# TobyBoyne/bark

Measured on AMD Instinct MI355X. Metric: forest-Gram + Cholesky MLL evals/sec at N=4096, 50 trees, higher is better.
Workload: dtype f64; 1 GPU; c3: N=4096 d=8 m=50, 256 prior forest samples per GPU (BASELINE configs[2]; sharding of configs[3]), noise U[0.05,0.15), mcmc_record_mll convention; N=4096, d=8, trees=50, forests_per_gpu=256, forests_total=256, chunk=256, parallelism=samples/1, launched_by=bench.py, device_wait=on

## Files before the change

### bark_amd/csrc/chol.hip

```cpp
#include <atomic>
#include <cmath>
#include <cstdlib>
#include <mutex>
#include <type_traits>
#include <vector>

#include "common.h"

namespace bark {

int walk_one_hot(const void *packed, const bark_pack_info *info, const double *X, int64_t N, int64_t d, int words,
                 uint32_t *out, int32_t *fault, hipStream_t stream);
int walk_codes(const void *packed, const bark_pack_info *info, const double *X, int64_t N, int64_t d, uint32_t *out,
               int32_t *fault, hipStream_t stream);
int leafspace_prepare(const uint32_t *codes, int W, int npad, unsigned long long *planes, int R, int Rpad,
                      const double *noise, const double *scale, int m, int bc, double *A, long ld, long bstride,
                      const double *y, int N, double *yz, double *accum, int32_t *info, hipStream_t s);
int leafspace_sumsq(const double *y, int N, double *out, hipStream_t s);
int leafspace_predict(const uint32_t *ccodes, int W, int cpad, int C, const double *w, const double *Minv, int R,
                      const double *noise, const double *scale, int m, int bc, double *mu, double *var, hipStream_t s);
int leafspace_inverse(const uint32_t *codes, int W, int npad, int N, const double *Minv, const double *w, int R,
                      const double *y, const double *noise, const double *scale, int m, int bc, double *Wm, double *kinv,
                      double *kinv_y, hipStream_t s);
int leafspace_finish(const double *accum, const double *yy, const double *noise, const double *scale, int m, int bc, int N,
// ... 58 lines not shown
#ifndef BARK_DIAG_WAVES8
#define BARK_DIAG_WAVES8 1
#endif
constexpr int DIAG8_MAX_BC = 256;
#ifndef BARK_WALK_IN_KERNEL
#define BARK_WALK_IN_KERNEL 1
#endif
#ifndef BARK_TWO_BLOCK
#define BARK_TWO_BLOCK 1
#endif
#ifndef BARK_TWO_MIN_BC
#define BARK_TWO_MIN_BC 1
#endif
constexpr int TWO_MIN_BC = BARK_TWO_MIN_BC, TWO_MAX_BC = 384, TWO_ANY_BC_MAX_N = 224;
#ifndef BARK_MULTI_BLOCK
#define BARK_MULTI_BLOCK 1
#endif
#ifndef BARK_MB_MIN_BC4
#define BARK_MB_MIN_BC4 112
#endif
#ifndef BARK_MB_MIN_BC3
#define BARK_MB_MIN_BC3 80
#endif
#ifndef BARK_MB_MIN_BC5
#define BARK_MB_MIN_BC5 144
#endif
constexpr int MB_MIN_BC4 = BARK_MB_MIN_BC4, MB_MIN_BC3 = BARK_MB_MIN_BC3, MB_MIN_BC5 = BARK_MB_MIN_BC5;
constexpr int MB_CUS = 256;
inline bool mb_chunk_ok(int nrb, int64_t bc) {
    const int64_t rounds = (bc + MB_CUS - 1) / MB_CUS;
    if (bc < (nrb <= 3 ? MB_MIN_BC3 : nrb == 4 ? MB_MIN_BC4 : MB_MIN_BC5)) return false;
    if (rounds <= 1) return true;
    return nrb <= 4 ? bc * 10 >= rounds * MB_CUS * 7 : bc * 5 >= rounds * MB_CUS * 4;
}
inline size_t mb_lds_bytes(int nW, int nrb) {
    return (size_t)(NBLK * SB * SB + 2 * NB + 8 + 2 * nrb * NB + 3 * MB_STAGE) * sizeof(double) + (size_t)nW * nrb * NB * sizeof(uint32_t);
}
#ifndef BARK_PIPE_MIN_NRB
#define BARK_PIPE_MIN_NRB 8
#endif
constexpr int PIPE_MIN_NRB = BARK_PIPE_MIN_NRB;
#ifndef BARK_PLAIN_CHUNK_MULTIPLE
#define BARK_PLAIN_CHUNK_MULTIPLE 256
#endif
constexpr int PLAIN_CHUNK_MULTIPLE = BARK_PLAIN_CHUNK_MULTIPLE;
#ifndef BARK_PLAIN_MIN_NRB
#define BARK_PLAIN_MIN_NRB 16
#endif
#ifndef BARK_PIPE_SYRK_MODE
#define BARK_PIPE_SYRK_MODE 2
#endif
#ifndef BARK_PLAIN_PAIRS
#define BARK_PLAIN_PAIRS 1
#endif
#ifndef BARK_PLAIN_SYRK_MODE
#define BARK_PLAIN_SYRK_MODE 2
#endif
constexpr int PLAIN_MIN_NRB = BARK_PLAIN_MIN_NRB;
#ifndef BARK_SOLVE_NARROW_MAX_WGS
#define BARK_SOLVE_NARROW_MAX_WGS 256
#endif
#ifndef BARK_PIPE_NARROW_MAX_WGS
#define BARK_PIPE_NARROW_MAX_WGS 256
#endif
constexpr long SOLVE_NARROW_MAX_WGS = BARK_SOLVE_NARROW_MAX_WGS, PIPE_NARROW_MAX_WGS = BARK_PIPE_NARROW_MAX_WGS;
#ifndef BARK_SOLVE_DIRECT_MAX_WGS
#define BARK_SOLVE_DIRECT_MAX_WGS 512
#endif
constexpr long SOLVE_DIRECT_MAX_WGS = BARK_SOLVE_DIRECT_MAX_WGS;

#ifndef BARK_DEVWAIT_MAX_BC
#define BARK_DEVWAIT_MAX_BC 32
#endif
constexpr int DEVWAIT_MAX_BC = BARK_DEVWAIT_MAX_BC;

struct Layout {
    int64_t npad, cpad, ncols, ld, W;
    bool splitk;
    size_t off_A, off_W, off_yz, off_acc, off_sync, off_leafx, off_leafc, off_slab, total;
};

inline size_t align256(size_t x) { return (x + 255) & ~(size_t)255; }

Layout make_layout(int64_t N, int64_t C, int64_t m, int64_t Bc) {
    Layout L;
    L.npad = round_up(N, NB);
    L.cpad = C > 0 ? round_up(C, NB) : 0;
    L.ncols = L.npad + L.cpad;
    L.ld = L.ncols + 16;
    L.W = MAX_LEAF_WORDS;
    size_t o = 0;
    L.off_A = o;
    o = align256(o + (size_t)Bc * L.npad * L.ld * sizeof(double));
    L.off_W = o;
    o = align256(o + (size_t)Bc * W_STRIDE * sizeof(double));
    L.off_yz = o;
    o = align256(o + (size_t)Bc * L.npad * sizeof(double));
    L.off_acc = o;
    o = align256(o + (size_t)Bc * 2 * sizeof(double));
    L.off_sync = o;
    o = align256(o + 64);
    L.off_leafx = o;
    o = align256(o + (size_t)Bc * L.W * L.npad * sizeof(uint32_t));
    L.off_leafc = o;
    o = align256(o + (size_t)Bc * L.W * L.cpad * sizeof(uint32_t));
    L.off_slab = o;
// ... 106 lines not shown
                if (hipEventRecord(res->rejoin[i], hs[i]) == hipSuccess) (void)hipStreamWaitEvent(main, res->rejoin[i], 0);
            }
        touched = 0;
        (void)hipGetLastError();
    }
    ~Sweep() {
        for (hipEvent_t e : ev) (void)hipEventDestroy(e);
    }

    int mark_on(hipStream_t s) {
        if (!timed) return BARK_OK;
        hipEvent_t e;
        BARK_HIP_CHECK(hipEventCreate(&e));
        ev.push_back(e);
        BARK_HIP_CHECK(hipEventRecord(e, s));
        return BARK_OK;
    }

    int launch_rows(hipStream_t st, int j, int kdone, int n_right, int n_tiles, int syrk) {
        if (syrk == 2 && n_tiles != n_right + 1) syrk = 0;
        const unsigned diag_wgs = (unsigned)(NXCD * ((p.Bc + NXCD - 1) / NXCD));
        const unsigned grid = syrk == 2 ? xcd_grid(n_right, p.Bc) + diag_wgs : xcd_grid(n_tiles, p.Bc);
        const dim3 g(grid), blk(THREADS);
        if (!fused)
            hipLaunchKernelGGL(row_kernel<0>, g, blk, GEMM_LDS, st, p, j, kdone, n_right, n_tiles, syrk);
        else if (rep == REP_BITS)
            hipLaunchKernelGGL(row_kernel<1 + REP_BITS>, g, blk, GEMM_LDS, st, p, j, kdone, n_right, n_tiles, syrk);
        else if (rep == REP_BYTES7)
            hipLaunchKernelGGL(row_kernel<1 + REP_BYTES7>, g, blk, GEMM_LDS, st, p, j, kdone, n_right, n_tiles, syrk);
        else
            hipLaunchKernelGGL(row_kernel<1 + REP_BYTES8>, g, blk, GEMM_LDS, st, p, j, kdone, n_right, n_tiles, syrk);
        BARK_LAUNCH_CHECK();
        panel_flops += 2.0 * NB * NB * (double)(kdone * NB) * ((double)n_right + (n_tiles > n_right ? (syrk ? 36.0 / 64.0 : 1.0) : 0.0)) * (double)p.Bc;
        return BARK_OK;
    }

    int launch_row_pair(hipStream_t st, int j) {
        const int nA = ncb - j - 1, nB = nA - 1, n_sq = nA + nB, n_syrk = 1 + ((j + 2 < nrb) ? 1 : 0);
        const unsigned grid = xcd_grid(n_sq, p.Bc) + (unsigned)(n_syrk * NXCD * ((p.Bc + NXCD - 1) / NXCD));
        const dim3 g(grid), blk(THREADS);
        if (!fused)
            hipLaunchKernelGGL(row_kernel<0>, g, blk, GEMM_LDS, st, p, j, j, nA, n_sq, 4);
        else if (rep == REP_BITS)
            hipLaunchKernelGGL(row_kernel<1 + REP_BITS>, g, blk, GEMM_LDS, st, p, j, j, nA, n_sq, 4);
        else if (rep == REP_BYTES7)
            hipLaunchKernelGGL(row_kernel<1 + REP_BYTES7>, g, blk, GEMM_LDS, st, p, j, j, nA, n_sq, 4);
        else
            hipLaunchKernelGGL(row_kernel<1 + REP_BYTES8>, g, blk, GEMM_LDS, st, p, j, j, nA, n_sq, 4);
        BARK_LAUNCH_CHECK();
        panel_flops += 2.0 * NB * NB * (double)(j * NB) * ((double)n_sq + n_syrk * 36.0 / 64.0) * (double)p.Bc;
        return BARK_OK;
    }

    int step_paired(int j) {
        hipStream_t s = main, ps = panel;
        const int bc = p.Bc, n_right = ncb - j - 1;
        const bool even = (j & 1) == 0, pair = even && j + 1 < nrb;
        int r;
        const bool has_rows = even && (pair || n_right > 0) && (j >= 1 || fused);
        if (has_rows) {
            BARK_HIP_CHECK(hipEventRecord(res->events[6 * j], s));
            if ((r = after(ps, res->events[6 * j]))) return r;
        }
        const int nkb = j == 0 ? 0 : (even ? 2 : 1);
        const bool deferred = !even;
        if ((r = launch_diag(j, nkb, deferred && n_right > 0, -2, j + 1))) return r;
        if (has_rows) {
            if (timed) panel_marks.push_back(ev.size());
            if ((r = mark_on(ps))) return r;
            if (pair) {
                if ((r = launch_row_pair(ps, j))) return r;
            } else if ((r = launch_rows(ps, j, j, n_right, n_right, 0))) {
                return r;
            }
            if ((r = mark_on(ps))) return r;
            if ((r = join(6 * j + 1))) return r;
        }
        if (n_right > 0) {
            if (timed) solve_marks.push_back(ev.size());
            if ((r = mark_on(s))) return r;
            const dim3 g(xcd_grid(n_right, bc)), blk(THREADS);
            if (deferred)
                hipLaunchKernelGGL(solve_kernel<1>, g, blk, GEMM_LDS, s, p, j, n_right);
            else
                hipLaunchKernelGGL(solve_kernel<0>, g, blk, GEMM_LDS, s, p, j, n_right);
            BARK_LAUNCH_CHECK();
            if ((r = mark_on(s))) return r;
            solve_flops += ((deferred ? 32.0 : 0.0) + 18.0) / 32.0 * 2.0 * NB * NB * (double)NB * (double)n_right * (double)bc;
        }
        return BARK_OK;
    }

    int publish(hipStream_t st, int slot, int value) {
        touch(st);
        hipLaunchKernelGGL(sync_publish_kernel, dim3(1), dim3(1), 0, st, p.sync, slot, value);
        BARK_LAUNCH_CHECK();
        return BARK_OK;
    }

    int gate(hipStream_t st, int value) {
        touch(st);
        hipLaunchKernelGGL(sync_gate_kernel, dim3(1), dim3(1), 0, st, p.sync, 3, value);
        BARK_LAUNCH_CHECK();
        return BARK_OK;
    }

    bool walk_in_kernel(const bark_pack_info *sub, int64_t d) const {
        return BARK_WALK_IN_KERNEL && nrb == 1 && BARK_DIAG_WAVES8 && p.Bc <= DIAG8_MAX_BC &&
               ((size_t)p.N * (d | 1) + 2 + (size_t)sub->m * sub->stride * 2) * sizeof(double) <= (size_t)NBLK * SB * SB * sizeof(double);
    }
    int launch_one_block(const double *y, double *mll, int32_t *fault, int include_2pi, const void *packed_c, const bark_pack_info *sub,
                         const double *X, int64_t d) {
        OneBlock ob{y, mll, fault, include_2pi, rep};
        if (walk_in_kernel(sub, d)) {
            ob.nodes = static_cast<const uint4 *>(packed_c);
            ob.X = X;
            ob.fault_w = fault;
            ob.stride = (int)sub->stride;
            ob.m = (int)sub->m;
            ob.max_depth = (int)sub->max_depth;
            ob.d = (int)d;
        }
        const size_t lds_bytes = DIAG_LDS + (size_t)p.nW * NB * sizeof(uint32_t);
        const bool w8 = BARK_DIAG_WAVES8 && p.Bc <= DIAG8_MAX_BC;
        if (nrb >= 3) {
            hipLaunchKernelGGL(multi_block_kernel, dim3((unsigned)p.Bc), dim3(512), mb_lds_bytes(p.nW, nrb), main, p, ob);
        } else if (nrb == 2) {
            const size_t lds2 = DIAG_LDS + (size_t)p.nW * 2 * NB * sizeof(uint32_t) + 2 * NB * sizeof(double);
            if (w8)
                hipLaunchKernelGGL(two_block_kernel<8>, dim3((unsigned)p.Bc), dim3(512), lds2, main, p, ob);
            else
                hipLaunchKernelGGL(two_block_kernel<4>, dim3((unsigned)p.Bc), dim3(THREADS), lds2, main, p, ob);
        } else if (w8) {
            hipLaunchKernelGGL((diag_kernel<true, 8>), dim3((unsigned)p.Bc), dim3(512), lds_bytes, main, p, 0, 0, 0, -2, 0, ob, 0);
        } else {
            hipLaunchKernelGGL((diag_kernel<true, 4>), dim3((unsigned)p.Bc), dim3(THREADS), lds_bytes, main, p, 0, 0, 0, -2, 0, ob, 0);
        }
        BARK_LAUNCH_CHECK();
        return BARK_OK;
    }

    int launch_diag(int j, int nkb, int want_g = 0, int wait_slot = -2, int wait_value = 0) {
        int r;
        if (timed) diag_marks.push_back(ev.size());
        if ((r = mark_on(main))) return r;
        const bool exclusive = p.Bc <= DIAG_EXCLUSIVE_MAX_BC && !lookahead(j + 1);
        int publish = wait_slot >= -1 ? 1 : 0;
        if (pre_update && nkb > 0) {
            hipLaunchKernelGGL(diag_pre_kernel, dim3(NBLK / (THREADS / 64), (unsigned)p.Bc), dim3(THREADS), 0, main, p, j, nkb, publish);
            BARK_LAUNCH_CHECK();
            nkb = 0;
            publish = 0;
        }
        const OneBlock fin = (fin_mll && j == nrb_steps - 1 && wait_slot < 0) ? OneBlock{nullptr, fin_mll, fin_fault, fin_2pi, rep} : OneBlock{};
        if (fin.mll) finished = true;
        if (exclusive && BARK_DIAG_WAVES8)
            hipLaunchKernelGGL((diag_kernel<false, 8>), dim3((unsigned)p.Bc), dim3(512), DIAG_LDS_EXCLUSIVE, main, p, j, nkb, want_g, wait_slot,
                               wait_value, fin, publish);
        else
            hipLaunchKernelGGL((diag_kernel<false, 4>), dim3((unsigned)p.Bc), dim3(THREADS), exclusive ? DIAG_LDS_EXCLUSIVE : DIAG_LDS, main, p, j, nkb,
                               want_g, wait_slot, wait_value, fin, publish);
        BARK_LAUNCH_CHECK();
        return mark_on(main);
    }

    int fork(int slot) {
        if (panel == main) return BARK_OK;
        BARK_HIP_CHECK(hipEventRecord(res->events[slot], main));
        return after(panel, res->events[slot]);
    }
    int join(int slot) {
        if (panel == main) return BARK_OK;
        BARK_HIP_CHECK(hipEventRecord(res->events[slot], panel));
        BARK_HIP_CHECK(hipStreamWaitEvent(main, res->events[slot], 0));
        joined(panel);
        return BARK_OK;
    }

    int split_factor(int j, int nkb, int slots = SPLITK_SLOTS) const {
        const int n_tiles = (ncb - j - 1) + ((j + 1 < nrb) ? 1 : 0);
        if (!splitk || j < 1 || n_tiles <= 0 || n_tiles * p.Bc >= SPLITK_SLOTS / 2 || nkb < 1) return 1;
        int S = slots / (n_tiles * p.Bc);
        if (slots != SPLITK_SLOTS) {
            S = (2 * slots + n_tiles * p.Bc) / (2 * n_tiles * p.Bc);
            while (S > 1 && S * n_tiles * p.Bc > SPLITK_SLOTS) --S;
        }
        if (S < 1) S = 1;
        int cap = nkb;
        if (slots == SPLITK_SLOTS && (long)n_tiles * p.Bc * nkb * SPLIT_FINE <= SPLIT_FINE_MAX_WGS) cap = nkb * SPLIT_FINE;
        if (S > cap) S = cap;
        if (S > SPLITK_MAX) S = SPLITK_MAX;
        return S;
    }
    bool lookahead(int j) const {
        if (la_stream == nullptr || j < 2 || j >= nrb_steps || split_factor(j, j) <= 1) return false;
        const long n_tiles = (ncb - j - 1) + ((j + 1 < nrb) ? 1 : 0);
        return n_tiles * p.Bc * (long)(j - 1) >= LA_MIN_WORK;
    }
    int la_slots(int j) const {
        const long n_tiles = (ncb - j - 1) + ((j + 1 < nrb) ? 1 : 0);
        return n_tiles * p.Bc * (long)(j - 1) >= LA_BULK_WORK ? LA_SLOTS : LA_SLOTS_CHAIN;
    }
    double *slab_set(int j) const { return slabs + (size_t)(j & 1) * SLAB_SET_TILES * NB * NB; }

    int launch_split(hipStream_t st, int j, int kb_lo, int kb_hi, int S, int s_off, int S_tot, int t_off = 0, int nt = -1) {
        const int n_right = ncb - j - 1, n_all = n_right + ((j + 1 < nrb) ? 1 : 0);
        if (nt < 0) nt = n_all - t_off;
        hipLaunchKernelGGL(panel_split_kernel, dim3(xcd_grid(nt * S, p.Bc)), dim3(THREADS), GEMM_LDS, st, p, j, n_right, t_off, nt,
                           kb_lo, kb_hi, S, s_off, S_tot, slab_set(j));
        BARK_LAUNCH_CHECK();
        panel_flops += 2.0 * NB * NB * (double)((kb_hi - kb_lo) * NB) * (double)nt * (double)p.Bc;
        return BARK_OK;
    }
// ... 806 lines not shown
```

### bark_amd/csrc/chol_diag.h

```cpp
#pragma once
#include <type_traits>

#include "chol_tiles.h"

namespace bark {
namespace {

constexpr int SB = 16;
constexpr int NSB = NB / SB;
constexpr int NBLK = NSB * (NSB + 1) / 2;
constexpr int NSB_ROWS = NSB;

__device__ __forceinline__ int blk_off(int rb, int cb) { return (rb * NSB - (rb * (rb - 1)) / 2 + (cb - rb)) * SB * SB; }
__device__ __forceinline__ double &s_at(double *S, int r, int c) {
    return S[blk_off(r >> 4, c >> 4) + (r & 15) * SB + (c & 15)];
}

__device__ __forceinline__ void mfma_tn(f64x4 &acc, const double *X, int ldx, const double *Y, int ldy, int lr, int lk) {
#pragma unroll
    for (int kk = 0; kk < SB / 4; ++kk)
        acc = __builtin_amdgcn_mfma_f64_16x16x4f64(X[(kk * 4 + lk) * ldx + lr], Y[(kk * 4 + lk) * ldy + lr], acc, 0, 0, 0);
}
__device__ __forceinline__ void mfma_nn(f64x4 &acc, const double *X, int ldx, const double *Y, int ldy, int lr, int lk) {
#pragma unroll
// ... 326 lines not shown
                for (int blk = 0; blk < 8; ++blk)
                    if (blk >= W) fr[blk] = st[(kk * 4 + lk) * LDS_LD + blk * 16 + lr];
#pragma unroll
                for (int i = LO; i < HI; ++i) acc[i] = __builtin_amdgcn_mfma_f64_16x16x4f64(fr[T::rb[i]], fr[T::cb[i]], acc[i], 0, 0, 0);
            }
            asm volatile("s_waitcnt vmcnt(0)" ::: "memory");
            __syncthreads();
        }
    }
#pragma unroll
    for (int i = LO; i < HI; ++i) {
        double *blk = S + blk_off(T::rb[i], T::cb[i]);
#pragma unroll
        for (int v = 0; v < 4; ++v) blk[(lk + 4 * v) * SB + lr] = pre[i][v] - acc[i][v];
    }
}

__device__ __forceinline__ void diag_g(const double *__restrict__ Up, long ld, const double *S, double *__restrict__ Gb, int wave_u,
                                    int lr, int lk) {
#pragma unroll 1
    for (int h = 0; h < 2; ++h) {
        const int kr = wave_u * 2 + h;
        const double *urow = Up + (size_t)(kr * SB + lr) * ld + lk;
        f64x4 g[NSB];
#pragma unroll
        for (int cbk = 0; cbk < NSB; ++cbk) g[cbk] = (f64x4){0.0, 0.0, 0.0, 0.0};
        double a[4], an[4];
#pragma unroll
        for (int q4 = 0; q4 < 4; ++q4) a[q4] = urow[q4 * 4];
#pragma unroll
        for (int rbk = 0; rbk < NSB; ++rbk) {
            if (rbk + 1 < NSB) {
#pragma unroll
                for (int q4 = 0; q4 < 4; ++q4) an[q4] = urow[(rbk + 1) * SB + q4 * 4];
            }
#pragma unroll
            for (int cbk = rbk; cbk < NSB; ++cbk) {
                const double *wb = S + blk_off(rbk, cbk);
#pragma unroll
                for (int q4 = 0; q4 < 4; ++q4)
                    g[cbk] = __builtin_amdgcn_mfma_f64_16x16x4f64(a[q4], wb[(q4 * 4 + lk) * SB + lr], g[cbk], 0, 0, 0);
            }
#pragma unroll
            for (int q4 = 0; q4 < 4; ++q4) a[q4] = an[q4];
            __builtin_amdgcn_sched_barrier(0);
        }
#pragma unroll
        for (int cbk = 0; cbk < NSB; ++cbk)
#pragma unroll
            for (int v = 0; v < 4; ++v) Gb[(size_t)(kr * SB + lk + 4 * v) * NB + cbk * SB + lr] = -g[cbk][v];
    }
}

__device__ __forceinline__ f64x4 frag_transpose(const f64x4 &a, int lr, int lk) {
    f64x4 d = {0.0, 0.0, 0.0, 0.0};
#pragma unroll
    for (int kk = 0; kk < SB / 4; ++kk) d = __builtin_amdgcn_mfma_f64_16x16x4f64(a[kk], (lk + 4 * kk == lr) ? 1.0 : 0.0, d, 0, 0, 0);
    return d;
}

template <int L>
__device__ __forceinline__ f64x4 x_entry(f64x4 (&xt)[L], f64x4 &tacc, int rb, int kb, int nsb, const double *S, const double *dblk,
                                         int lr, int lk) {
    auto term = [&](f64x4 &t, int k, int col, const f64x4 &xf) {
        const double *ub = S + blk_off(k, col);
#pragma unroll
        for (int kk = 0; kk < SB / 4; ++kk) t = __builtin_amdgcn_mfma_f64_16x16x4f64(ub[(kk * 4 + lk) * SB + lr], xf[kk], t, 0, 0, 0);
    };
    if (kb == rb + 1) {
        const double *w = S + blk_off(rb, rb);
        f64x4 wk;
#pragma unroll
        for (int v = 0; v < 4; ++v) wk[v] = w[(lk + 4 * v) * SB + lr];
        xt[0] = frag_transpose(wk, lr, lk);
        tacc = (f64x4){0.0, 0.0, 0.0, 0.0};
    }
    f64x4 t = tacc;
#pragma unroll
    for (int d = 0; d < L; ++d)
        if (rb + d == kb - 1) term(t, kb - 1, kb, xt[d]);
    f64x4 x = {0.0, 0.0, 0.0, 0.0};
#pragma unroll
    for (int kk = 0; kk < SB / 4; ++kk) x = __builtin_amdgcn_mfma_f64_16x16x4f64(dblk[(kk * 4 + lk) * SB + lr], t[kk], x, 0, 0, 0);
    x = -x;
#pragma unroll
    for (int d = 1; d < L; ++d)
        if (rb + d == kb) xt[d] = x;
    if (kb + 1 < nsb) {
        f64x4 tn = {0.0, 0.0, 0.0, 0.0};
#pragma unroll
        for (int d = 0; d < L; ++d)
            if (rb + d < kb) term(tn, rb + d, kb + 1, xt[d]);
        tacc = tn;
    }
    return x;
}

template <int Q, int STRIDE = 3>
__device__ __forceinline__ void c_group(double *S, int kb, int n, int i0, int lr, int lk) {
    const double *a[Q], *b[Q];
    double *dd[Q];
#pragma unroll
    for (int qq = 0; qq < Q; ++qq) {
        int r = 0, rem = i0 + STRIDE * qq + 1;
        while (rem >= n - r) {
            rem -= n - r;
// ... 327 lines not shown
        const double *prev = Ab + (size_t)(j - nkb) * NB * p.ld + (size_t)j * NB;
        const int wsel = __builtin_amdgcn_readfirstlane(wave);
        if (ONE && NW == 8) {
            switch (wsel) {
                case 0: mb_update<0, 0, 5>(prev, p.ld, 0, lds, S, wsel, lane, q.lr, q.lk, p, b, ob.rep, codes, NB, 0); break;
                case 1: mb_update<1, 0, 5>(prev, p.ld, 0, lds, S, wsel, lane, q.lr, q.lk, p, b, ob.rep, codes, NB, 0); break;
                case 2: mb_update<2, 0, 5>(prev, p.ld, 0, lds, S, wsel, lane, q.lr, q.lk, p, b, ob.rep, codes, NB, 0); break;
                case 3: mb_update<3, 0, 5>(prev, p.ld, 0, lds, S, wsel, lane, q.lr, q.lk, p, b, ob.rep, codes, NB, 0); break;
                case 4: mb_update<0, 5, 9>(prev, p.ld, 0, lds, S, wsel, lane, q.lr, q.lk, p, b, ob.rep, codes, NB, 0); break;
                case 5: mb_update<1, 5, 9>(prev, p.ld, 0, lds, S, wsel, lane, q.lr, q.lk, p, b, ob.rep, codes, NB, 0); break;
                case 6: mb_update<2, 5, 9>(prev, p.ld, 0, lds, S, wsel, lane, q.lr, q.lk, p, b, ob.rep, codes, NB, 0); break;
                default: mb_update<3, 5, 9>(prev, p.ld, 0, lds, S, wsel, lane, q.lr, q.lk, p, b, ob.rep, codes, NB, 0); break;
            }
        } else if (wsel == 0)
            diag_update<0, ONE>(tile, p.ld, prev, nkb, lds, S, lane, q.lr, q.lk, p, b, ob.rep, codes);
        else if (wsel == 1)
            diag_update<1, ONE>(tile, p.ld, prev, nkb, lds, S, lane, q.lr, q.lk, p, b, ob.rep, codes);
        else if (wsel == 2)
            diag_update<2, ONE>(tile, p.ld, prev, nkb, lds, S, lane, q.lr, q.lk, p, b, ob.rep, codes);
        else if (NW == 4 || wsel == 3)
            diag_update<3, ONE>(tile, p.ld, prev, nkb, lds, S, lane, q.lr, q.lk, p, b, ob.rep, codes);
        else
            for (int a = (nkb > 1 ? 2 : nkb) * (1 + NB / BK); a > 0; --a) __syncthreads();
    }
    __syncthreads();

    const int lr = q.lr, lk = q.lk;
    const int wave_u = __builtin_amdgcn_readfirstlane(wave);
    const int nsb = one ? (p.N + SB - 1) / SB : NSB;
    DIAG_STAMP(1);
    if (NW == 8)
        factor_tile8<ONE>(S, nsb, copy_only, wave_u, lane, lr, lk, logsum, pacc, bad);
    else
        factor_tile<ONE>(S, nsb, copy_only, wave_u, lane, lr, lk, logsum, pacc, bad);
    DIAG_STAMP(2);

    double *Wb = w_block(p, b);
    auto write_w = [&](int t) {
        const int half = __builtin_amdgcn_readfirstlane(t >> 7), e = 2 * (t & 127), r = e >> 4, c = e & 15;
        int cnt = 0;
#pragma unroll
        for (int rbk = 0; rbk < NSB; ++rbk)
#pragma unroll
            for (int cbk = rbk; cbk < NSB; ++cbk, ++cnt)
                if ((cnt & 1) == half)
                    *reinterpret_cast<f64x2 *>(Wb + (size_t)(rbk * SB + r) * NB + cbk * SB + c) =
                        *reinterpret_cast<const f64x2 *>(S + blk_off(rbk, cbk) + e);
    };
    if (!one && NW == 4) write_w(tid);

    DIAG_STAMP(3);
    if (want_g && (NW == 4 || wave_u < 4))
        diag_g(Ab + (size_t)(j - 1) * NB * p.ld + (size_t)j * NB, p.ld, S, p.W + (size_t)b * W_STRIDE, wave_u, lr, lk);

    DIAG_STAMP(4);
    double *yb = p.yz + (size_t)b * p.nrb * NB + (size_t)j * NB;
    if (tid < NB) vec[tid] = y_in;
    __syncthreads();
    {
        const int c = tid & (NB - 1), half = tid >> 7, cbk = c >> 4, cc = c & 15;
        double part = 0.0;
#pragma unroll
        for (int i = 0; i < NSB / 2; ++i) {
            const int rbk = half * (NSB / 2) + i;
            if (rbk <= cbk && (NW == 4 || half < 2)) {
                const double *col = S + blk_off(rbk, cbk) + cc;
#pragma unroll
                for (int rr = 0; rr < SB; ++rr) part = fma(col[rr * SB], vec[rbk * SB + rr], part);
            }
        }
        if (half == 1) vec[NB + c] = part;
        __syncthreads();
        double zz = 0.0;
        if (!half) {
            const double z = part + vec[NB + c];
            if (!one) yb[c] = z;
            zz = z * z;
        }
#pragma unroll
        for (int off = 32; off > 0; off >>= 1) zz += __shfl_xor(zz, off);
        if (lane == 0) red[wave] = zz;
    }
    __syncthreads();
    DIAG_STAMP(5);
    if (!one && NW == 8 && tid >= THREADS) write_w(tid - THREADS);
    if (tid == 0 && one) {
        double v = -(red[0] + red[1]) - 2.0 * logsum;
        if (ob.include_2pi) v = v - (double)p.N * log(2.0 * M_PI);
        ob.mll[b] = 0.5 * v;
        p.info[b] = *ob.fault ? -1 : (bad ? bad : 0);
    } else if (tid == 0) {
        p.accum[(size_t)b * 2 + 0] = acc_quad + (red[0] + red[1]);
        p.accum[(size_t)b * 2 + 1] = acc_logdet + 2.0 * logsum;
        int code = (bad && info_in == 0) ? j * NB + bad : 0;
        if (wait_slot >= 0) {
            const unsigned long long t0 = __builtin_amdgcn_s_memrealtime();
            const int32_t *flag = p.sync + wait_slot;
            bool ok = true;
            while (__hip_atomic_load(flag, __ATOMIC_RELAXED, __HIP_MEMORY_SCOPE_AGENT) < wait_value) {
                if (__hip_atomic_load(p.sync + 2, __ATOMIC_RELAXED, __HIP_MEMORY_SCOPE_AGENT) != 0) {
                    ok = false;
                    break;
                }
                __builtin_amdgcn_s_sleep(8);
                if (__builtin_amdgcn_s_memrealtime() - t0 > 200000000ull) {
                    ok = false;
// ... 411 lines not shown
```

### bark_amd/csrc/chol_solve.h

```cpp
#pragma once
#include "chol_rows.h"

namespace bark {
namespace {

template <int DEF>
__global__ __launch_bounds__(THREADS, 2) void solve_kernel(Mats p, int j, int n_right) {
    extern __shared__ __attribute__((aligned(16))) double lds[];
    const int tid = threadIdx.x;
    int b, t;
    if (!xcd_map(blockIdx.x, n_right, p.Bc, b, t)) return;
    const Lane q = lane_of(tid);
    const int cb = j + 1 + t;
    double *Ab = p.A + (size_t)b * p.bstride;
    double *tile = Ab + (size_t)j * NB * p.ld + (size_t)cb * NB;
    const double *Pb = p.W + (size_t)b * W_STRIDE + (size_t)(1 - DEF) * NB * NB;

    f64x4 acc[4][4];
    zero_acc(acc);
    const int wr_u = __builtin_amdgcn_readfirstlane(q.wr);
    const int rt[4] = {wr_u ? 1 : 0, wr_u ? 2 : 3, wr_u ? 5 : 4, wr_u ? 6 : 7};
    gemm_upper_tri<DEF>(acc, rt, Pb, tile - (size_t)DEF * NB * p.ld, p.ld, lds, tid, q);
#pragma unroll
    for (int mt = 0; mt < 4; ++mt)
#pragma unroll
        for (int v = 0; v < 4; ++v) {
            double *row = tile + (size_t)(rt[mt] * 16 + q.lk + 4 * v) * p.ld;
#pragma unroll
            for (int nt = 0; nt < 4; ++nt) row[acc_col(q, nt)] = acc[mt][nt][v];
        }
    if (cb >= p.nrb) return;

    double *part = lds;
    const double *zb = p.yz + (size_t)b * p.nrb * NB + (size_t)j * NB;
#pragma unroll
    for (int mt = 0; mt < 4; ++mt) y_partial<4>(acc[mt], rt[mt], zb, part, q.wc * 64, q);
    __syncthreads();
    if (tid < NB) y_commit(part, p.yz + (size_t)b * p.nrb * NB + (size_t)cb * NB, tid);
}

template <int NT, int DEF = 0>
__global__ __launch_bounds__(THREADS, 2) void solve_narrow_kernel(Mats p, int j, int n_right) {
    constexpr int PARTS = 4 / NT, WCOLS = 32 * NT, nd = DEF * (NB / BK), nk = nd + NB / BK;
    extern __shared__ __attribute__((aligned(16))) double lds[];
    const int tid = threadIdx.x;
    int b, tp;
    if (!xcd_map(blockIdx.x, n_right * PARTS, p.Bc, b, tp)) return;
    const Lane q = lane_of(tid);
    const int t = tp / PARTS, c_off = (tp - t * PARTS) * WCOLS + q.wc * 16 * NT;
    const int cb = j + 1 + t;
    double *tile = p.A + (size_t)b * p.bstride + (size_t)j * NB * p.ld + (size_t)cb * NB;
    const double *Wb = p.W + (size_t)b * W_STRIDE + (size_t)(1 - DEF) * NB * NB;
    const double *Tp = tile - (size_t)DEF * NB * p.ld;
    const int wr_u = __builtin_amdgcn_readfirstlane(q.wr);
    const int rt[4] = {wr_u ? 1 : 0, wr_u ? 2 : 3, wr_u ? 5 : 4, wr_u ? 6 : 7};
    f64x4 acc[4][NT];
#pragma unroll
    for (int mt = 0; mt < 4; ++mt)
#pragma unroll
        for (int nt = 0; nt < NT; ++nt) acc[mt][nt] = (f64x4){0.0, 0.0, 0.0, 0.0};
    const int wave = __builtin_amdgcn_readfirstlane(tid >> 6), lane = tid & 63;
    stage_dma(Wb, NB, Tp, p.ld, 0, lds, wave, lane);
    asm volatile("s_waitcnt vmcnt(0)" ::: "memory");
    __syncthreads();
#pragma unroll
    for (int kt = 0; kt < nk; ++kt) {
        if (kt + 1 < nk) stage_dma(Wb, NB, Tp, p.ld, kt + 1, lds + ((kt + 1) & 1) * STAGE, wave, lane);
        const double *As = lds + (kt & 1) * STAGE;
        const double *Bs = As + BK * LDS_LD;
#pragma unroll
        for (int kk = 0; kk < BK / 4; ++kk) {
            double bf[NT];
#pragma unroll
            for (int nt = 0; nt < NT; ++nt) bf[nt] = Bs[(kk * 4 + q.lk) * LDS_LD + c_off + nt * 16 + q.lr];
#pragma unroll
            for (int mt = 0; mt < 4; ++mt) {
                if (kt < nd || kt - nd <= rt[mt]) {
                    const double a = As[(kk * 4 + q.lk) * LDS_LD + rt[mt] * 16 + q.lr];
#pragma unroll
                    for (int nt = 0; nt < NT; ++nt)
                        acc[mt][nt] = __builtin_amdgcn_mfma_f64_16x16x4f64(a, bf[nt], acc[mt][nt], 0, 0, 0);
                }
            }
        }
        asm volatile("s_waitcnt vmcnt(0)" ::: "memory");
        __syncthreads();
    }
#pragma unroll
    for (int mt = 0; mt < 4; ++mt)
#pragma unroll
        for (int v = 0; v < 4; ++v) {
// ... 228 lines not shown
```

### bark_amd/csrc/chol_tiles.h

```cpp
#pragma once
#include "common.h"

namespace bark {
namespace {

#ifdef BARK_DIAG_STAMPS
__device__ unsigned long long g_diag_stamps[64];
#define DIAG_STAMP(i) do { if (blockIdx.x == 0 && threadIdx.x == 0) g_diag_stamps[i] = __builtin_readcyclecounter(); } while (0)
#else
#define DIAG_STAMP(i) do {} while (0)
#endif

typedef double f64x4 __attribute__((ext_vector_type(4)));
typedef double f64x2 __attribute__((ext_vector_type(2)));

constexpr int NB = TILE;
constexpr int BK = 16;
constexpr int LDS_LD = NB + 16;
constexpr int STAGE = 2 * BK * LDS_LD;
constexpr int GEMM_LDS_DOUBLES = 2 * STAGE;
constexpr int THREADS = 256;

struct Lane {
    int wr, wc, lr, lk;
// ... 117 lines not shown
#pragma unroll
            for (int mt = 0; mt < 4; ++mt) {
                if (kw <= rt[mt]) {
                    const double a = As[(kk * 4 + q.lk) * LDS_LD + rt[mt] * 16 + q.lr];
                    acc[mt][0] = __builtin_amdgcn_mfma_f64_16x16x4f64(a, b0, acc[mt][0], 0, 0, 0);
                    acc[mt][1] = __builtin_amdgcn_mfma_f64_16x16x4f64(a, b1, acc[mt][1], 0, 0, 0);
                    acc[mt][2] = __builtin_amdgcn_mfma_f64_16x16x4f64(a, b2, acc[mt][2], 0, 0, 0);
                    acc[mt][3] = __builtin_amdgcn_mfma_f64_16x16x4f64(a, b3, acc[mt][3], 0, 0, 0);
                }
            }
        }
        asm volatile("s_waitcnt vmcnt(0)" ::: "memory");
        __syncthreads();
    }
}

constexpr int NXCD = 8;
__host__ __device__ __forceinline__ int xcd_rep(int Bc) {
    const int rounds = (Bc + NXCD - 1) / NXCD;
    if (Bc % NXCD == 0 || (Bc > NXCD && rounds * NXCD * 10 < Bc * 11)) return 1;
    return (Bc % 4 == 0) ? 2 : (Bc % 2 == 0) ? 4 : 8;
}
__host__ __device__ __forceinline__ bool xcd_map(int id, int ntiles, int Bc, int &b, int &tile) {
    const int R = xcd_rep(Bc), ntv = (ntiles + R - 1) / R;
    const int x = id % NXCD, q = id / NXCD;
    const int v = (q / ntv) * NXCD + x;
    b = v / R;
    tile = (q % ntv) * R + (v - b * R);
    return b < Bc && tile < ntiles;
}
__host__ __device__ inline unsigned xcd_grid(int ntiles, int Bc) {
    const int R = xcd_rep(Bc), ntv = (ntiles + R - 1) / R;
    return (unsigned)(NXCD * ((Bc * R + NXCD - 1) / NXCD) * ntv);
}

struct Mats {
    double *A;
    long ld, bstride;
    double *W;
    double *yz;
    double *accum;
    int32_t *info;
    int nrb;
    int ncb;
    int Bc;
    const uint32_t *leafx;
    const double *scale;
    const double *shift;
    const double *noise;
    int nW, m, N;
    int32_t *sync;
};

constexpr size_t W_STRIDE = (size_t)2 * NB * NB;
__device__ __forceinline__ double *w_block(const Mats &p, int b) { return p.W + (size_t)b * W_STRIDE + (size_t)NB * NB; }

}
}
```

Baseline: 2813 evals/s.

## Fuse paired-step triangular solves into one two-row-block solve kernel

For paired Cholesky steps, the even step now stores its inverse factor in a shifted W slot and skips its per-tile solve. The odd step's diagonal kernel additionally computes a product H of the saved inverse with G. A new pair_solve_kernel then updates both block rows of each right-hand tile in a single pass, producing both the j-1 and j rows and their y contributions. This is meant to cut the number of solve launches and dependent passes over the trailing panel. In exchange it grows the per-batch W workspace from two to three blocks and adds extra MFMA work in the diagonal kernel.

```diff
diff --git a/bark_amd/csrc/chol.hip b/bark_amd/csrc/chol.hip
--- a/bark_amd/csrc/chol.hip
+++ b/bark_amd/csrc/chol.hip
@@ -134,6 +134,9 @@
 #endif
 #ifndef BARK_PLAIN_PAIRS
 #define BARK_PLAIN_PAIRS 1
+#endif
+#ifndef BARK_PAIR_SOLVE
+#define BARK_PAIR_SOLVE 1
 #endif
 #ifndef BARK_PLAIN_SYRK_MODE
 #define BARK_PLAIN_SYRK_MODE 2
@@ -346,6 +349,11 @@
         return BARK_OK;
     }
 
+    Mats w_saved() const {
+        Mats q = p;
+        q.W += (size_t)NB * NB;
+        return q;
+    }
     int step_paired(int j) {
         hipStream_t s = main, ps = panel;
         const int bc = p.Bc, n_right = ncb - j - 1;
@@ -358,7 +366,9 @@
         }
         const int nkb = j == 0 ? 0 : (even ? 2 : 1);
         const bool deferred = !even;
-        if ((r = launch_diag(j, nkb, deferred && n_right > 0, -2, j + 1))) return r;
+        const bool pair_solve = BARK_PAIR_SOLVE != 0;
+        const int want_g = deferred && n_right > 0 ? (pair_solve ? 2 : 1) : 0;
+        if ((r = launch_diag(j, nkb, want_g, -2, j + 1, pair_solve && pair))) return r;
         if (has_rows) {
             if (timed) panel_marks.push_back(ev.size());
             if ((r = mark_on(ps))) return r;
@@ -373,14 +383,22 @@
         if (n_right > 0) {
             if (timed) solve_marks.push_back(ev.size());
             if ((r = mark_on(s))) return r;
-            const dim3 g(xcd_grid(n_right, bc)), blk(THREADS);
-            if (deferred)
-                hipLaunchKernelGGL(solve_kernel<1>, g, blk, GEMM_LDS, s, p, j, n_right);
-            else
-                hipLaunchKernelGGL(solve_kernel<0>, g, blk, GEMM_LDS, s, p, j, n_right);
+            const dim3 blk(THREADS);
+            if (pair_solve && pair) {
+                hipLaunchKernelGGL(solve_direct_kernel<0>, dim3(xcd_grid(8, bc)), blk, 0, s, w_saved(), j, 1);
+            } else if (pair_solve && deferred) {
+                hipLaunchKernelGGL(pair_solve_kernel, dim3(xcd_grid(2 * n_right, bc)), blk, PAIR_LDS_DOUBLES * sizeof(double), s, p, j - 1,
+                                   n_right);
+            } else if (deferred) {
+                hipLaunchKernelGGL(solve_kernel<1>, dim3(xcd_grid(n_right, bc)), blk, GEMM_LDS, s, p, j, n_right);
+            } else {
+                hipLaunchKernelGGL(solve_kernel<0>, dim3(xcd_grid(n_right, bc)), blk, GEMM_LDS, s, p, j, n_right);
+            }
             BARK_LAUNCH_CHECK();
             if ((r = mark_on(s))) return r;
-            solve_flops += ((deferred ? 32.0 : 0.0) + 18.0) / 32.0 * 2.0 * NB * NB * (double)NB * (double)n_right * (double)bc;
+            const double tiles = pair_solve && pair ? 1.0 : (double)n_right;
+            const double per_tile = pair_solve && deferred ? 68.0 : (deferred ? 50.0 : 18.0);
+            solve_flops += per_tile / 32.0 * 2.0 * NB * NB * (double)NB * tiles * (double)bc;
         }
         return BARK_OK;
     }
@@ -434,8 +452,9 @@
         return BARK_OK;
     }
 
-    int launch_diag(int j, int nkb, int want_g = 0, int wait_slot = -2, int wait_value = 0) {
+    int launch_diag(int j, int nkb, int want_g = 0, int wait_slot = -2, int wait_value = 0, bool w_saved_w = false) {
         int r;
+        const Mats pd = w_saved_w ? w_saved() : p;
         if (timed) diag_marks.push_back(ev.size());
         if ((r = mark_on(main))) return r;
         const bool exclusive = p.Bc <= DIAG_EXCLUSIVE_MAX_BC && !lookahead(j + 1);
@@ -449,10 +468,10 @@
         const OneBlock fin = (fin_mll && j == nrb_steps - 1 && wait_slot < 0) ? OneBlock{nullptr, fin_mll, fin_fault, fin_2pi, rep} : OneBlock{};
         if (fin.mll) finished = true;
         if (exclusive && BARK_DIAG_WAVES8)
-            hipLaunchKernelGGL((diag_kernel<false, 8>), dim3((unsigned)p.Bc), dim3(512), DIAG_LDS_EXCLUSIVE, main, p, j, nkb, want_g, wait_slot,
+            hipLaunchKernelGGL((diag_kernel<false, 8>), dim3((unsigned)p.Bc), dim3(512), DIAG_LDS_EXCLUSIVE, main, pd, j, nkb, want_g, wait_slot,
                                wait_value, fin, publish);
         else
-            hipLaunchKernelGGL((diag_kernel<false, 4>), dim3((unsigned)p.Bc), dim3(THREADS), exclusive ? DIAG_LDS_EXCLUSIVE : DIAG_LDS, main, p, j, nkb,
+            hipLaunchKernelGGL((diag_kernel<false, 4>), dim3((unsigned)p.Bc), dim3(THREADS), exclusive ? DIAG_LDS_EXCLUSIVE : DIAG_LDS, main, pd, j, nkb,
                                want_g, wait_slot, wait_value, fin, publish);
         BARK_LAUNCH_CHECK();
         return mark_on(main);
diff --git a/bark_amd/csrc/chol_diag.h b/bark_amd/csrc/chol_diag.h
--- a/bark_amd/csrc/chol_diag.h
+++ b/bark_amd/csrc/chol_diag.h
@@ -402,6 +402,40 @@
     }
 }
 
+template <int NW>
+__device__ __forceinline__ void diag_h(double *Gn, const double *__restrict__ Wp, int wave_u, int lr, int lk) {
+    constexpr int RPW = 8 / NW;
+    __syncthreads();
+    f64x4 h[RPW][NSB];
+#pragma unroll
+    for (int i = 0; i < RPW; ++i) {
+        const int rb = wave_u * RPW + i;
+#pragma unroll
+        for (int cbk = 0; cbk < NSB; ++cbk) h[i][cbk] = (f64x4){0.0, 0.0, 0.0, 0.0};
+#pragma unroll 1
+        for (int kb = rb; kb < NSB; ++kb) {
+            double a[4];
+#pragma unroll
+            for (int q4 = 0; q4 < 4; ++q4) a[q4] = Wp[(size_t)(rb * SB + lr) * NB + kb * SB + q4 * 4 + lk];
+#pragma unroll
+            for (int cbk = 0; cbk < NSB; ++cbk) {
+                const double *g = Gn + (size_t)(kb * SB + lk) * NB + cbk * SB + lr;
+#pragma unroll
+                for (int q4 = 0; q4 < 4; ++q4) h[i][cbk] = __builtin_amdgcn_mfma_f64_16x16x4f64(a[q4], g[(size_t)(q4 * 4) * NB], h[i][cbk], 0, 0, 0);
+            }
+        }
+    }
+    __syncthreads();
+#pragma unroll
+    for (int i = 0; i < RPW; ++i) {
+        const int rb = wave_u * RPW + i;
+#pragma unroll
+        for (int cbk = 0; cbk < NSB; ++cbk)
+#pragma unroll
+            for (int v = 0; v < 4; ++v) Gn[(size_t)(rb * SB + lk + 4 * v) * NB + cbk * SB + lr] = h[i][cbk][v];
+    }
+}
+
 __device__ __forceinline__ f64x4 frag_transpose(const f64x4 &a, int lr, int lk) {
     f64x4 d = {0.0, 0.0, 0.0, 0.0};
 #pragma unroll
@@ -835,6 +869,8 @@
     DIAG_STAMP(3);
     if (want_g && (NW == 4 || wave_u < 4))
         diag_g(Ab + (size_t)(j - 1) * NB * p.ld + (size_t)j * NB, p.ld, S, p.W + (size_t)b * W_STRIDE, wave_u, lr, lk);
+    if (want_g == 2)
+        diag_h<NW>(p.W + (size_t)b * W_STRIDE, p.W + (size_t)b * W_STRIDE + (size_t)2 * NB * NB, wave_u, lr, lk);
 
     DIAG_STAMP(4);
     double *yb = p.yz + (size_t)b * p.nrb * NB + (size_t)j * NB;
diff --git a/bark_amd/csrc/chol_solve.h b/bark_amd/csrc/chol_solve.h
--- a/bark_amd/csrc/chol_solve.h
+++ b/bark_amd/csrc/chol_solve.h
@@ -37,6 +37,123 @@
     for (int mt = 0; mt < 4; ++mt) y_partial<4>(acc[mt], rt[mt], zb, part, q.wc * 64, q);
     __syncthreads();
     if (tid < NB) y_commit(part, p.yz + (size_t)b * p.nrb * NB + (size_t)cb * NB, tid);
+}
+
+constexpr int PBK = 8;
+constexpr int PSTAGE = 2 * PBK * LDS_LD + (PBK / 2) * LDS_LD;
+constexpr int PAIR_LDS_DOUBLES = 2 * PSTAGE;
+
+__device__ __forceinline__ void pair_stage(const double *__restrict__ A1, const double *__restrict__ A2, const double *__restrict__ T,
+                                           long ld, double *st, int wave, int lane) {
+    double *a1s = st, *a2s = st + PBK * LDS_LD, *bs = st + 2 * PBK * LDS_LD;
+    dma_row(A1 + (long)wave * NB + lane * 2, a1s + wave * LDS_LD);
+    dma_row(A1 + (long)(wave + 4) * NB + lane * 2, a1s + (wave + 4) * LDS_LD);
+    if (A2) {
+        dma_row(A2 + (long)wave * NB + lane * 2, a2s + wave * LDS_LD);
+        dma_row(A2 + (long)(wave + 4) * NB + lane * 2, a2s + (wave + 4) * LDS_LD);
+    }
+    dma_row(T + (long)(wave + 4 * (lane >> 5)) * ld + (lane & 31) * 2, bs + wave * LDS_LD);
+}
+
+__global__ __launch_bounds__(THREADS, 2) void pair_solve_kernel(Mats p, int j, int n_right) {
+    extern __shared__ __attribute__((aligned(16))) double lds[];
+    const int tid = threadIdx.x;
+    int b, tp;
+    if (!xcd_map(blockIdx.x, n_right * 2, p.Bc, b, tp)) return;
+    const Lane q = lane_of(tid);
+    const int cb = j + 2 + (tp >> 1), col0 = (tp & 1) * 64;
+    double *tile = p.A + (size_t)b * p.bstride + (size_t)j * NB * p.ld + (size_t)cb * NB + col0;
+    const double *Wm = p.W + (size_t)b * W_STRIDE;
+    const double *Hn = Wm, *W1 = Wm + (size_t)NB * NB, *W0 = Wm + (size_t)2 * NB * NB;
+    const int wave = __builtin_amdgcn_readfirstlane(tid >> 6), lane = tid & 63;
+    const int rt[2] = {wave, 7 - wave};
+    f64x4 acc[4][4];
+    zero_acc(acc);
+    constexpr int NKH = NB / PBK;
+    pair_stage(W0, Hn, tile, p.ld, lds, wave, lane);
+    asm volatile("s_waitcnt vmcnt(0)" ::: "memory");
+    __syncthreads();
+    for (int kt = 0; kt < NKH; ++kt) {
+        const int kn = kt + 1;
+        if (kn < NKH)
+            pair_stage(W0 + (size_t)kn * PBK * NB, Hn + (size_t)kn * PBK * NB, tile + (size_t)kn * PBK * p.ld, p.ld, lds + (kn & 1) * PSTAGE,
+                       wave, lane);
+        else
+            pair_stage(W1, nullptr, tile + (size_t)kn * PBK * p.ld, p.ld, lds + (kn & 1) * PSTAGE, wave, lane);
+        const double *A1s = lds + (kt & 1) * PSTAGE, *A2s = A1s + PBK * LDS_LD, *Bs = A2s + PBK * LDS_LD;
+        const int kb = kt / (16 / PBK);
+#pragma unroll
+        for (int kk = 0; kk < PBK / 4; ++kk) {
+            const double *br = Bs + q.lk * LDS_LD + kk * 64 + q.lr;
+            const double b0 = br[0], b1 = br[16], b2 = br[32], b3 = br[48];
+            const double *ar = A1s + (kk * 4 + q.lk) * LDS_LD + q.lr, *hr = A2s + (kk * 4 + q.lk) * LDS_LD + q.lr;
+#pragma unroll
+            for (int h = 0; h < 2; ++h) {
+                if (kb <= rt[h]) {
+                    const double a = ar[rt[h] * 16];
+                    acc[h][0] = __builtin_amdgcn_mfma_f64_16x16x4f64(a, b0, acc[h][0], 0, 0, 0);
+                    acc[h][1] = __builtin_amdgcn_mfma_f64_16x16x4f64(a, b1, acc[h][1], 0, 0, 0);
+                    acc[h][2] = __builtin_amdgcn_mfma_f64_16x16x4f64(a, b2, acc[h][2], 0, 0, 0);
+                    acc[h][3] = __builtin_amdgcn_mfma_f64_16x16x4f64(a, b3, acc[h][3], 0, 0, 0);
+                }
+                const double a = hr[rt[h] * 16];
+                acc[2 + h][0] = __builtin_amdgcn_mfma_f64_16x16x4f64(a, b0, acc[2 + h][0], 0, 0, 0);
+                acc[2 + h][1] = __builtin_amdgcn_mfma_f64_16x16x4f64(a, b1, acc[2 + h][1], 0, 0, 0);
+                acc[2 + h][2] = __builtin_amdgcn_mfma_f64_16x16x4f64(a, b2, acc[2 + h][2], 0, 0, 0);
+                acc[2 + h][3] = __builtin_amdgcn_mfma_f64_16x16x4f64(a, b3, acc[2 + h][3], 0, 0, 0);
+            }
+        }
+        asm volatile("s_waitcnt vmcnt(0)" ::: "memory");
+        __syncthreads();
+    }
+    for (int kt = 0; kt < NKH; ++kt) {
+        const int kn = kt + 1;
+        if (kn < NKH)
+            pair_stage(W1 + (size_t)kn * PBK * NB, nullptr, tile + (size_t)(NKH + kn) * PBK * p.ld, p.ld, lds + ((NKH + kn) & 1) * PSTAGE, wave,
+                       lane);
+        const double *A1s = lds + ((NKH + kt) & 1) * PSTAGE, *Bs = A1s + 2 * PBK * LDS_LD;
+        const int kb = kt / (16 / PBK);
+#pragma unroll
+        for (int kk = 0; kk < PBK / 4; ++kk) {
+            const double *br = Bs + q.lk * LDS_LD + kk * 64 + q.lr;
+            const double b0 = br[0], b1 = br[16], b2 = br[32], b3 = br[48];
+            const double *ar = A1s + (kk * 4 + q.lk) * LDS_LD + q.lr;
+#pragma unroll
+            for (int h = 0; h < 2; ++h) {
+                if (kb <= rt[h]) {
+                    const double a = ar[rt[h] * 16];
+                    acc[2 + h][0] = __builtin_amdgcn_mfma_f64_16x16x4f64(a, b0, acc[2 + h][0], 0, 0, 0);
+                    acc[2 + h][1] = __builtin_amdgcn_mfma_f64_16x16x4f64(a, b1, acc[2 + h][1], 0, 0, 0);
+                    acc[2 + h][2] = __builtin_amdgcn_mfma_f64_16x16x4f64(a, b2, acc[2 + h][2], 0, 0, 0);
+                    acc[2 + h][3] = __builtin_amdgcn_mfma_f64_16x16x4f64(a, b3, acc[2 + h][3], 0, 0, 0);
+                }
+            }
+        }
+        asm volatile("s_waitcnt vmcnt(0)" ::: "memory");
+        __syncthreads();
+    }
+#pragma unroll
+    for (int mt = 0; mt < 4; ++mt)
+#pragma unroll
+        for (int v = 0; v < 4; ++v) {
+            double *row = tile + (size_t)((mt >> 1) * NB + rt[mt & 1] * 16 + q.lk + 4 * v) * p.ld;
+#pragma unroll
+            for (int nt = 0; nt < 4; ++nt) row[nt * 16 + q.lr] = acc[mt][nt][v];
+        }
+    if (cb >= p.nrb) return;
+    double *part0 = lds, *part1 = lds + NSB_ROWS * NB;
+    const double *zb = p.yz + (size_t)b * p.nrb * NB + (size_t)j * NB;
+#pragma unroll
+    for (int h = 0; h < 2; ++h) {
+        y_partial<4>(acc[h], rt[h], zb, part0, 0, q);
+        y_partial<4>(acc[2 + h], rt[h], zb + NB, part1, 0, q);
+    }
+    __syncthreads();
+    if (tid < 64) {
+        double *yi = p.yz + (size_t)b * p.nrb * NB + (size_t)cb * NB + col0;
+        y_commit(part0, yi, tid);
+        y_commit(part1, yi, tid);
+    }
 }
 
 template <int NT, int DEF = 0>
diff --git a/bark_amd/csrc/chol_tiles.h b/bark_amd/csrc/chol_tiles.h
--- a/bark_amd/csrc/chol_tiles.h
+++ b/bark_amd/csrc/chol_tiles.h
@@ -193,7 +193,7 @@
     int32_t *sync;
 };
 
-constexpr size_t W_STRIDE = (size_t)2 * NB * NB;
+constexpr size_t W_STRIDE = (size_t)3 * NB * NB;
 __device__ __forceinline__ double *w_block(const Mats &p, int b) { return p.W + (size_t)b * W_STRIDE + (size_t)NB * NB; }
 
 }
```

New measurement: 2791 evals/s, median of 2. No clear change (-0.8%).
